# wenxichen/tensorflow_yolo2

Hardware: AMD Instinct MI355X
Metric: images/sec fwd+bwd Darknet-19 416x416 (higher is better)
Workload: dtype f16; 1 GPU; YOLO detector train step: darknet19_core + darknet19_detection(30) + get_loss + backward + Adam; image_size=416, batch_per_gpu=64, global_batch=64, S=13, B=2, parallelism=dp1, grad_allreduce=none

## Files before the change

include/yolo2_hip.h:

```cpp
#ifndef YOLO2_HIP_H
#define YOLO2_HIP_H
#include <stddef.h>
#include <stdint.h>

#ifdef __cplusplus
extern "C" {
#endif
#pragma GCC visibility push(default)

typedef struct y2_ctx y2_ctx;

#define Y2_F32 0
#define Y2_F16 1
#define Y2_BF16 2
#define Y2_F16X2 3
#define Y2_F16X2F 4
#define Y2_FP8 5

#define Y2_TAIL_NONE 0
#define Y2_TAIL_AVGPOOL 1

#define Y2_OK 0
#define Y2_ERR_ARG -1
#define Y2_ERR_HIP -2
// ... 177 lines not shown
int y2_momentum_step_packed(y2_ctx* ctx, float* accum, void* ctrl, float lr, float momentum, float grad_mult,
                            void* stream);

#define Y2_POLICY_CONSTANT 0
#define Y2_POLICY_STEPS 1
#define Y2_POLICY_POLY 2
#define Y2_SOLVER_MAX_STEPS 8
typedef struct y2_sgd_solver {
    float learning_rate, momentum, decay;
    int policy, burn_in, power, max_batches, nsteps;
    int steps[Y2_SOLVER_MAX_STEPS];
    float scales[Y2_SOLVER_MAX_STEPS];
} y2_sgd_solver;
int y2_solver_rate(const y2_sgd_solver* solver, int t, float* rate);
int y2_sgd_step(y2_ctx* ctx, float* accum, void* ctrl, int step, const y2_sgd_solver* solver, float grad_mult,
                void* stream);
int y2_sgd_step_packed(y2_ctx* ctx, float* accum, void* ctrl, int step, const y2_sgd_solver* solver, float grad_mult,
                       void* stream);

int y2_backward_adam(y2_ctx* ctx, const float* dout, float* m, float* v, void* ctrl, int step, float lr, float beta1,
                     float beta2, float eps, float grad_mult, void* stream);
int y2_backward_momentum(y2_ctx* ctx, const float* dout, float* accum, void* ctrl, float lr, float momentum,
                         float grad_mult, void* stream);

size_t y2_conv2d_workspace_bytes(int N, int H, int W, int Cin, int Cout, int k, int dtype);
int y2_conv2d(const float* x, const float* w, const float* bias, float* y, int N, int H, int W, int Cin,
              int Cout, int k, int dtype, void* workspace, void* stream);
int y2_conv2d_backward(const float* x, const float* w, const float* dy, float* dx, float* dw, int N, int H,
                       int W, int Cin, int Cout, int k, int dtype, void* workspace, void* stream);

#define Y2_LAUNCH_LOG_INTS 7
int y2_launch_log_enable(int enable);
int y2_launch_log_read(int* out, int max_records);

int y2_mx_quantize(const float* x, size_t rows, int C, uint8_t* q, uint8_t* scales, void* stream);

#define Y2_RESIZE_MAX_OUT_W 1024
int y2_resize_bilinear_u8_batch(const uint8_t* pool, const int64_t* table, const int32_t* index, int n, int out_h,
                                int out_w, uint8_t* out, void* stream);
int y2_letterbox_geometry(int im_h, int im_w, int size, int* geometry);
int y2_letterbox_u8_batch(const uint8_t* pool, const int64_t* table, const int32_t* index, int n, int size, int fill,
                          uint8_t* out, void* stream);
int y2_encode_labels(const double* boxes, const int32_t* counts, const int64_t* table, const int32_t* index, int n,
                     int max_obj, int image_size, int S, int num_class, float* labels, void* stream);

int y2_augment_u8_batch(const uint8_t* pool, const int64_t* table, const int32_t* index, const double* params, int n,
// ... 71 lines not shown
```

tensorflow_yolo2_amd/_lib.py:

```python
import ctypes as C
import os

_HERE = os.path.dirname(os.path.abspath(__file__))
LIB_PATH = os.path.join(_HERE, "libyolo2_hip.so")
if os.environ.get("Y2_DEV_LIB") == "1":
    LIB_PATH = os.path.join(_HERE, "libyolo2_hip_dev.so")
if os.environ.get("Y2_LIB_PATH"):
    LIB_PATH = os.environ["Y2_LIB_PATH"]

Y2_F32, Y2_F16, Y2_BF16, Y2_F16X2, Y2_F16X2F, Y2_FP8 = 0, 1, 2, 3, 4, 5
LOSS_SCALED = (Y2_F16, Y2_F16X2, Y2_F16X2F)
Y2_TAIL_NONE, Y2_TAIL_AVGPOOL = 0, 1
LAUNCH_LOG_INTS = 7
DTYPES = {"f32": Y2_F32, "fp32": Y2_F32, "float32": Y2_F32,
          "f16": Y2_F16, "fp16": Y2_F16, "float16": Y2_F16,
          "bf16": Y2_BF16, "bfloat16": Y2_BF16,
          "f16x2": Y2_F16X2,
          "f16x2f": Y2_F16X2F,
          "fp8": Y2_FP8, "mxfp8": Y2_FP8}

_vp, _i, _f, _sz, _u64 = C.c_void_p, C.c_int, C.c_float, C.c_size_t, C.c_uint64
_pi = C.POINTER(C.c_int)
_psz = C.POINTER(C.c_size_t)

# ... 91 lines not shown
    "y2_fully_connected_backward": (_i, [_vp, _vp, _vp, _vp, _vp, _i, _i, _i, _i, _vp]),
    "y2_conv7x7s2": (_i, [_vp, _vp, _vp, _i, _i, _i, _i, _vp]),
    "y2_conv7x7s2_t": (_i, [_vp, _vp, _vp, _i, _i, _i, _i, _i, _vp]),
    "y2_conv7x7s2_backward_filter": (_i, [_vp, _vp, _vp, _i, _i, _i, _i, _vp]),
    "y2_conv7x7s2_backward_filter_t": (_i, [_vp, _vp, _vp, _i, _i, _i, _i, _i, _vp]),
    "y2_bias_relu": (_i, [_vp, _vp, _sz, _i, _i, _vp]),
    "y2_bias_relu_backward": (_i, [_vp, _vp, _vp, _vp, _sz, _i, _i, _vp]),
    "y2_dropout": (_i, [_vp, _vp, _sz, _f, _u64, _vp]),
    "y2_dropout_dev": (_i, [_vp, _vp, _sz, _f, _vp, _vp]),
    "y2_adam_step": (_i, [_vp, _vp, _vp, _vp, _sz, _i, _f, _f, _f, _f, _f, _vp]),
    "y2_momentum_step": (_i, [_vp, _vp, _vp, _sz, _f, _f, _f, _vp]),
    "y2_grad_check": (_i, [_vp, _vp, _vp]),
    "y2_grad_check_more": (_i, [_vp, _vp, _vp]),
    "y2_grad_check_full": (_i, [_vp, _sz, _vp, _vp]),
    "y2_adam_step_guarded": (_i, [_vp, _vp, _vp, _vp, _sz, _vp, _f, _f, _f, _f, _f, _vp]),
    "y2_momentum_step_guarded": (_i, [_vp, _vp, _vp, _sz, _vp, _f, _f, _f, _vp]),
    "y2_adam_step_packed": (_i, [_vp, _vp, _vp, _vp, _i, _f, _f, _f, _f, _f, _vp]),
    "y2_momentum_step_packed": (_i, [_vp, _vp, _vp, _f, _f, _f, _vp]),
    "y2_solver_rate": (_i, [_vp, _i, C.POINTER(C.c_float)]),
    "y2_sgd_step": (_i, [_vp, _vp, _vp, _i, _vp, _f, _vp]),
    "y2_sgd_step_packed": (_i, [_vp, _vp, _vp, _i, _vp, _f, _vp]),
    "y2_backward_adam": (_i, [_vp, _vp, _vp, _vp, _vp, _i, _f, _f, _f, _f, _f, _vp]),
    "y2_backward_momentum": (_i, [_vp, _vp, _vp, _vp, _f, _f, _f, _vp]),
    "y2_conv2d_workspace_bytes": (_sz, [_i, _i, _i, _i, _i, _i, _i]),
    "y2_conv2d": (_i, [_vp, _vp, _vp, _vp, _i, _i, _i, _i, _i, _i, _i, _vp, _vp]),
    "y2_conv2d_backward": (_i, [_vp, _vp, _vp, _vp, _vp, _i, _i, _i, _i, _i, _i, _i, _vp, _vp]),
    "y2_launch_log_enable": (_i, [_i]),
    "y2_launch_log_read": (_i, [_pi, _i]),
    "y2_mx_quantize": (_i, [_vp, _sz, _i, _vp, _vp, _vp]),
    "y2_resize_bilinear_u8_batch": (_i, [_vp, _vp, _vp, _i, _i, _i, _vp, _vp]),
    "y2_letterbox_geometry": (_i, [_i, _i, _i, _pi]),
    "y2_letterbox_u8_batch": (_i, [_vp, _vp, _vp, _i, _i, _i, _vp, _vp]),
    "y2_encode_labels": (_i, [_vp, _vp, _vp, _vp, _i, _i, _i, _i, _i, _vp, _vp]),
    "y2_augment_u8_batch": (_i, [_vp, _vp, _vp, _vp, _i, _i, _i, _i, _vp, _vp]),
    "y2_encode_labels_window": (_i, [_vp, _vp, _vp, _vp, _vp, _i, _i, _i, _i, _i, _vp, _vp]),
    "y2_encode_box_list": (_i, [_vp, _vp, _vp, _vp, _vp, _i, _i, _i, _i, _vp, _vp, _vp]),
    "y2_encode_box_list_draw": (_i, [_vp, _vp, _vp, _vp, _vp, _vp, _i, _i, _i, _i, _vp, _vp, _vp]),
    "y2_warp_u8_batch": (_i, [_vp, _vp, _vp, _vp, _vp, _i, _i, _i, _i, _vp, _vp, _vp]),
    "y2_detect_grid_batch": (_i, [_vp, _vp, _vp, _i, _i, _i, _i, _f, _f, _i, _vp, _vp, _vp, _vp]),
    "y2_detect_anchor_batch": (_i, [_vp, _vp, _vp, _vp, _i, _i, _i, _i, _f, _f, _i, _vp, _vp, _vp, _vp]),
    "y2_detect_anchor_batch_lb": (_i, [_vp, _vp, _vp, _vp, _i, _i, _i, _i, _f, _f, _i, _i, _vp, _vp, _vp, _vp]),
    "y2_detect_anchor_classes_batch": (_i, [_vp, _vp, _vp, _vp, _i, _i, _i, _i, _f, _f, _i, _vp, _vp, _vp, _vp]),
    "y2_detect_anchor_classes_batch_lb": (_i, [_vp, _vp, _vp, _vp, _i, _i, _i, _i, _f, _f, _i, _i, _vp, _vp, _vp, _vp]),
    "y2_voc_match_batch": (_i, [_vp, _vp, _vp, _vp, _vp, _vp, _vp, _i, _i, _i, _f, _vp, _vp]),
    "y2_letterbox_darknet_batch": (_i, [_vp, _vp, _vp, _i, _i, _vp, _vp]),
    "y2_detect_anchor_classes_batch_dk": (_i, [_vp, _vp, _vp, _vp, _i, _i, _i, _i, _f, _f, _i, _i, _vp, _vp, _vp, _vp]),
# ... 62 lines not shown
```

tensorflow_yolo2_amd/csrc/kernels.h:

```cpp
#pragma once
#include <hip/hip_runtime.h>
#include <stddef.h>
#include <stdint.h>
#include <atomic>
#include "../../include/yolo2_hip.h"

namespace y2 {

inline size_t dtype_size(int dtype) { return (dtype == 0 || dtype >= 3) ? 4 : 2; }
inline int dtype_kbytes(int dtype) { return dtype == 0 ? 4 : 2; }
inline bool dtype_split(int dtype) { return dtype >= 3; }
inline int dtype_plain(int dtype) { return dtype >= 3 ? 0 : dtype; }

struct ConvArgs {
    const void* x;
    const void* w;
    void* y;
    const float* bias;
    float* part_cnt;
    float* part_mean;
    float* part_m2;
    int N, H, W, C;
    int M;
    int Cout;
// ... 357 lines not shown
hipError_t launch_pack_input_u8(int dtype, const uint8_t* img, void* x4, int N, int H, int W, hipStream_t s);
hipError_t launch_pack_weights(int dtype, const float* W, void* wf, void* wd, int taps, int Cin, int Cout,
                               int Cout_pad, int Kc, int Cin_pad, int Cdy, int frag, hipStream_t s);
hipError_t launch_pack_conv1_weights(int dtype, const float* W, void* wp, hipStream_t s);
struct PackLayer {
    const float* W;
    size_t w_off;
    void* wf;
    void* wd;
    int taps, Cin, Cout, Cout_pad, Kc, Cin_pad, Cdy;
    int wf_bx, wf_by, wf_blocks, wd_blocks, first_block;
    int opt_first;
    int wf_frag, wd_frag;
};
void pack_layer_plan(PackLayer& L, int first_block, int elem_size);
hipError_t launch_pack_all(int dtype, const PackLayer* tab_dev, int nlayers, int total_blocks, hipStream_t s);
struct OptPackArgs {
    float* p; float* slot0; float* slot1; const float* g;
    const void* ctrl;
    float lr_t, b1, b2, eps, gmult;
    int kind;
    const PackLayer* tab; int nlayers; int tile_blocks;
    const unsigned* small; int nsmall;
};
hipError_t launch_opt_pack(int dtype, const OptPackArgs& a, hipStream_t s);
hipError_t launch_convert_grad(int dtype, const float* src, void* dst, int M, int C, int ldd, float scale,
                               hipStream_t s);
hipError_t launch_unpack_act(int dtype, const void* xp, float* out, int N, int H, int W, int C, int Cs,
                             hipStream_t s);
hipError_t launch_pack_act_region(int dtype, const float* in, void* region, size_t region_bytes, size_t front_px, int N,
                                  int H, int W, int C, int Cs, hipStream_t s);
hipError_t launch_pack_act(int dtype, const float* in, void* xp, int N, int H, int W, int C, int Cs,
                           hipStream_t s);
hipError_t launch_cast_to_f32(int dtype, const void* src, float* dst, size_t rows, int C, int lds, hipStream_t s,
                              float scale = 1.0f);

struct BnFinalizeArgs {
    const float* part_cnt;
    const float* part_mean;
    const float* part_m2;
    int P, C, ldp;
    const float* gamma;
    const float* beta;
    float* moving_mean;
    float* moving_var;
    float* scale;
// ... 78 lines not shown
    float lambda_coord, lambda_noobj;
};
int loss_blocks(int N, int S);
hipError_t launch_yolo_loss(const LossArgs& a, hipStream_t s);
hipError_t launch_get_iou(const float* b1, const float* b2, float* out, int n, hipStream_t s);
hipError_t launch_decode(const float* pred, int S, int B, int C, int im_w, int im_h, float thresh, int* out,
                         float* out_conf, hipStream_t s);
hipError_t launch_avgpool_fwd(const float* h, float* out, int N, int H, int W, int C, int k, hipStream_t s);
hipError_t launch_avgpool_bwd(const float* dout, float* dh, int N, int H, int W, int C, int k, hipStream_t s);
hipError_t launch_softmax_ce(const float* logits, const int* labels, float* loss, float* dlogits, int N, int C,
                             hipStream_t s);

hipError_t launch_accuracy(const float* logits, const int* labels, float* acc, int N, int C, hipStream_t s);

hipError_t launch_adam(float* p, float* m, float* v, const float* g, size_t n, float lr_t, float b1, float b2,
                       float eps, float gscale, hipStream_t s);
hipError_t launch_momentum(float* p, float* acc, const float* g, size_t n, float lr, float mom, float gscale,
                           hipStream_t s);
hipError_t launch_grad_check(const float* g, size_t n, void* ctrl, hipStream_t s);
hipError_t launch_grad_check_ranges(const float* g, const void* ranges_dev, int nranges, void* ctrl, hipStream_t s,
                                    unsigned* flag = nullptr, bool keep = false);
hipError_t launch_range_check(const float* x, size_t n, float limit, void* ctrl, hipStream_t s);
hipError_t launch_opt_ctrl_advance(void* ctrl, float lr, float b1, float b2, hipStream_t s);
hipError_t launch_adam_guarded(float* p, float* m, float* v, const float* g, size_t n, const void* ctrl, float b1,
                               float b2, float eps, float gscale, hipStream_t s);
hipError_t launch_momentum_guarded(float* p, float* acc, const float* g, size_t n, const void* ctrl, float lr, float mom,
                                   float gscale, hipStream_t s);
struct SgdSeg { unsigned off, cnt, first_block, decayed; };
int sgd_seg_blocks(size_t off, size_t cnt);
hipError_t launch_sgd(float* p, float* acc, const float* g, const SgdSeg* segs_dev, int nsegs, int blocks,
                      const void* ctrl, float lr_t, float mom, float decay, float gscale, hipStream_t s);
hipError_t launch_sgd_ctrl_advance(void* ctrl, const y2_sgd_solver& sv, hipStream_t s);
hipError_t launch_init_trunc_normal(float* p, size_t n, float stddev, uint64_t seed, uint64_t stream_id,
                                    hipStream_t s);
hipError_t launch_fill(float* p, size_t n, float v, hipStream_t s);

constexpr int kDetectMaxCand = Y2_DETECT_MAX_CANDIDATES;
constexpr int kDetectAnchorMaxCand = Y2_DETECT_ANCHOR_MAX_CANDIDATES;
constexpr int kMatchMaxObj = Y2_MATCH_MAX_OBJECTS;

void* op_scratch(hipStream_t s, size_t bytes);
int op_scratch_error();

}
```

tensorflow_yolo2_amd/csrc/net.hip:

```cpp
#include <math.h>
#include <stdarg.h>
#include <stdio.h>
#include <string.h>

#include <algorithm>
#include <string>
#include <vector>

#include "../../include/yolo2_hip.h"
#include "common.h"
#include "kernels.h"
#include "optim_math.h"

using namespace y2;

static thread_local std::string g_err;
namespace y2 {
int set_error(int code, const char* msg) {
    g_err = msg;
    return code;
}
}
static int fail(int code, const char* fmt, ...) {
    char buf[512];
// ... 129 lines not shown
    size_t o_ks = 0, ks_floats = 0;
    size_t o_gram = 0;
    size_t slab_floats = 0;
    int n_chkranges = 0, n_smallranges = 0, opt_tile_blocks = 0;
    int n_chk_upper = 0, n_small_upper = 0;
    int n_sgdsegs = 0, sgd_blocks = 0;
    struct FusedOpt {
        bool on = false;
        int kind = 0;
        float* slot0 = nullptr; float* slot1 = nullptr;
        void* ctrl = nullptr;
        float lr = 0.f, b1 = 0.f, b2 = 0.f, eps = 0.f, gmult = 1.f;
        int step = 0;
    } fopt;
    std::vector<PackLayer> packtab;
    std::vector<BnInferLayer> infertab;
    std::vector<SgdSeg> sgdsegs;
    int pack_blocks = 0;
    int prof = 0;
    struct ProfRec { int cat, layer; hipEvent_t a, b; };
    int prof_layer = -1;
    hipStream_t side = nullptr;
    hipEvent_t ev_fork = nullptr, ev_join = nullptr;
    std::vector<hipEvent_t> mark_main, mark_side;
    int n_marks = 0;
    const int* cur_marks = nullptr;
    float* dinput = nullptr;
    void* ext_xin = nullptr;
    void* ext_out = nullptr;
    const void* ext_join = nullptr;
    int ext_join_self = 0;
    const void* ext_dout = nullptr;
    void* ext_dx = nullptr;
    std::vector<ProfRec> prof_recs;
    size_t prof_used = 0;
    size_t sz() const { return dtype_size(dtype); }
    PadGeom in_geom(int l) const { return PadGeom{N, L[l].H, L[l].W, L[l].cin_s}; }
    PadGeom dy_geom(int l) const { return PadGeom{N, L[l].H, L[l].W, L[l].ldy}; }
    Conv1Plan conv1_plan(bool trains, bool training) const {
        const Layer& y = L[0];
        return plan_conv1(dtype, bwd_dtype, N, y.H, y.W, y.pool, y.cout, y.ldy, trains, L.size() > 1, training);
    }
};

enum { CAT_CONV_FWD = 0, CAT_CONV1_FWD, CAT_DGRAD, CAT_WGRAD, CAT_CONV1_WGRAD, CAT_BN_FWD, CAT_BN_BWD, CAT_MISC,
       CAT_COUNT };
// ... 381 lines not shown
        if (tail_k <= 0 || last.Ho < tail_k || last.Wo < tail_k) {
            delete c;
            return fail(Y2_ERR_ARG, "avgpool window %d does not fit %dx%d", tail_k, last.Ho, last.Wo);
        }
        c->outN = batch; c->outH = last.Ho / tail_k; c->outW = last.Wo / tail_k; c->outC = last.cout;
    } else {
        c->outN = batch; c->outH = last.Ho; c->outW = last.Wo; c->outC = last.cout;
    }
    if (last.pool) {
        delete c;
        return fail(Y2_ERR_ARG, "the last layer must not pool");
    }
    plan(c);
    *out = c;
    return Y2_OK;
}

void y2_ctx_destroy(y2_ctx* ctx) {
    if (!ctx) return;
    for (auto& r : ctx->prof_recs) { (void)hipEventDestroy(r.a); (void)hipEventDestroy(r.b); }
    if (ctx->side) (void)hipStreamDestroy(ctx->side);
    if (ctx->ev_fork) (void)hipEventDestroy(ctx->ev_fork);
    if (ctx->ev_join) (void)hipEventDestroy(ctx->ev_join);
    for (auto e : ctx->mark_main) (void)hipEventDestroy(e);
    for (auto e : ctx->mark_side) (void)hipEventDestroy(e);
    delete ctx;
}

int y2_profile_enable(y2_ctx* c, int on) {
    if (on == 1 || on == 2) c->prof_used = 0;
    c->prof = on == 3 ? 2 : on;
    return Y2_OK;
}
int y2_profile_collect(y2_ctx* c, double* ms, int* count, int ncat) {
    if (ncat < CAT_COUNT) return fail(Y2_ERR_ARG, "need room for %d categories", (int)CAT_COUNT);
    for (int i = 0; i < ncat; ++i) { ms[i] = 0.0; count[i] = 0; }
    for (size_t i = 0; i < c->prof_used; ++i) {
        auto& r = c->prof_recs[i];
        HIPCHK(hipEventSynchronize(r.b));
        float t = 0.f;
        HIPCHK(hipEventElapsedTime(&t, r.a, r.b));
        ms[r.cat] += t;
        count[r.cat] += 1;
    }
    c->prof_used = 0;
    return Y2_OK;
// ... 76 lines not shown
    c->packtab.clear();
    int nb = 0, ntile = 0;
    for (size_t l = 0; l < c->L.size(); ++l) {
        Layer& y = c->L[l];
        if (y.first3) continue;
        PackLayer p{};
        p.W = params + y.pW;
        p.w_off = y.pW;
        p.wf = c->ws + y.wf;
        p.wd = training ? (void*)(c->ws + y.wd) : nullptr;
        p.taps = y.k * y.k; p.Cin = y.cin; p.Cout = y.cout; p.Cout_pad = y.cout_pad; p.Kc = y.cin_s;
        p.Cin_pad = y.cin_pad; p.Cdy = y.ldy;
        const int split = dtype_split(c->dtype) ? 1 : 0;
        p.wf_frag = y.wf_frag = plan_conv(c->dtype, fwd_args(c, (int)l, false, FOLD_NONE)).filter_layout;
        p.wd_frag = y.wd_frag = plan_conv(dgrad_dtype(c, (int)l), dgrad_args(c, (int)l, false, false)).filter_layout;
        pack_layer_plan(p, nb, split ? 2 : (int)c->sz());
        nb += p.wf_blocks + p.wd_blocks;
        p.opt_first = ntile;
        ntile += p.wf_blocks;
        c->packtab.push_back(p);
    }
    c->pack_blocks = nb;
    c->opt_tile_blocks = ntile;
    {
        std::vector<unsigned> rg;
        for (size_t l = 1; l <= c->L.size(); ++l) {
            const Layer& y = c->L[l % c->L.size()];
            rg.push_back((unsigned)y.pb);
            rg.push_back((unsigned)(3 * y.cout));
            rg.push_back(0u);
        }
        c->n_small_upper = (int)c->L.size() - 1;
        if (c->L[0].first3) {
            rg.push_back((unsigned)c->L[0].pW);
            rg.push_back((unsigned)(27 * c->L[0].cout));
            rg.push_back(1u);
        }
        c->n_smallranges = (int)(rg.size() / 3);
        HIPCHK(hipMemcpyAsync(c->ws + c->o_smallranges, rg.data(), rg.size() * sizeof(unsigned), hipMemcpyHostToDevice,
                              (hipStream_t)stream));
    }
    {
        std::vector<SgdSeg>& sg = c->sgdsegs;
        sg.clear();
        unsigned nblk = 0;
        for (const Layer& y : c->L) {
// ... 302 lines not shown
        HIPCHK(launch_avgpool_fwd((const float*)(c->ws + c->o_h32), out, c->N, y.Ho, y.Wo, y.cout, c->tail_k, s));
    }
    c->fwd_saved = true;
    c->moving_pending = !update_moving;
    return Y2_OK;
}

int y2_update_moving_stats(y2_ctx* c, void* stream) {
    if (!c->ws) return fail(Y2_ERR_STATE, "bind buffers first");
    if (!c->fwd_saved) return fail(Y2_ERR_STATE, "run y2_forward first");
    if (!c->moving_pending) return Y2_OK;
    hipStream_t s = (hipStream_t)stream;
    for (size_t l = 0; l < c->L.size(); ++l) {
        if (!c->fwd.L[l].training) continue;
        const Layer& y = c->L[l];
        const float* stat = (const float*)(c->ws + y.stat);
        HIPCHK(launch_bn_update_moving(stat + 2 * y.ldy, stat + 6 * y.ldy, c->state + y.smm, c->state + y.smv, y.cout,
                                       c->bn_momentum, s));
    }
    c->moving_pending = false;
    return Y2_OK;
}

static int fused_opt_part(y2_ctx* c, int part, hipStream_t s);

int y2_backward(y2_ctx* c, const float* dout, int layer_lo, int layer_hi, void* stream) {
    if (c->fp8) return fail(Y2_ERR_STATE, "Y2_FP8 contexts are inference only: no backward pass (create the context with another dtype to train)");
    if (!c->ws || !c->bound_training) return fail(Y2_ERR_STATE, "bind with training=1 first");
    if (!c->fwd_saved) return fail(Y2_ERR_STATE, "run y2_forward before y2_backward");
    const int nl = (int)c->L.size();
    if (layer_lo < 0 || layer_hi > nl || layer_lo >= layer_hi) return fail(Y2_ERR_ARG, "bad layer range");
    hipStream_t s = (hipStream_t)stream;
    const size_t sz = c->sz();
    const float inv_gs = 1.0f / c->grad_scale;
    char* dA[2] = {c->ws + c->o_dA0, c->ws + c->o_dA1};
    const bool ext_top = layer_hi == nl && c->ext_dout != nullptr;
    if (layer_hi == nl) c->dA_half = 0;
    if (ext_top) {
        c->dA_cur = 0;
        if (layer_lo > 0 && c->grads) HIPCHK(hipMemsetAsync(c->grads, 0, c->L[layer_lo].pW * sizeof(float), s));
    } else if (layer_hi == nl) {
        if (!dout) return fail(Y2_ERR_ARG, "null output gradient");
        const Layer& y = c->L.back();
        const float* src = dout;
        if (c->tail == Y2_TAIL_AVGPOOL) {
            float* dh = (float*)(c->ws + c->o_dh32);
            HIPCHK(launch_avgpool_bwd(dout, dh, c->N, y.Ho, y.Wo, y.cout, c->tail_k, s));
            src = dh;
        }
        c->dA_cur = 0;
        PROF(CAT_MISC);
        HIPCHK(launch_convert_grad(c->dtype, src, dA[0], y.M, y.cout, y.ldy, c->grad_scale, s));
        if (layer_lo > 0 && c->grads) HIPCHK(hipMemsetAsync(c->grads, 0, c->L[layer_lo].pW * sizeof(float), s));
    }
    float* psum = (float*)(c->ws + c->o_psum);
    bool forked = false;
    bool opt_early = false;
    const NetPlan n = plan_net(c, c->fwd.train_core, c->fwd.train_head, layer_lo, layer_hi);
    const Conv1Plan& p1 = n.c1;
    if (!c->side && std::any_of(n.L.begin(), n.L.end(), [](const LayerPlan& p) { return p.wgrad_side; })) {
        HIPCHK(hipStreamCreateWithFlags(&c->side, hipStreamNonBlocking));
        HIPCHK(hipEventCreateWithFlags(&c->ev_fork, hipEventDisableTiming));
        HIPCHK(hipEventCreateWithFlags(&c->ev_join, hipEventDisableTiming));
    }
    for (int l = layer_hi - 1; l >= layer_lo; --l) {
        c->prof_layer = l;
        const Layer& y = c->L[l];
        const LayerPlan& p = n.L[l];
        float* stat = (float*)(c->ws + y.stat);
        char* dyp = c->ws + y.dyp + c->dy_geom(l).base_off(sz);
        BnBwdArgs b{};
        b.dA = (ext_top && l == nl - 1) ? c->ext_dout : (const void*)dA[c->dA_cur]; b.y = c->ws + y.y;
        b.scale = stat; b.shift = stat + y.ldy; b.mean = stat + 2 * y.ldy; b.invstd = stat + 3 * y.ldy;
        b.coef = stat + 4 * y.ldy;
        b.psum = psum;
        b.dgamma = c->grads + y.pg; b.dbeta = c->grads + y.pbeta; b.dbias = c->grads + y.pb;
        b.dyp = dyp;
        b.N = c->N; b.H = y.H; b.W = y.W; b.C = y.cout; b.ldy = y.ldy;
        b.ldd = y.ldy;
        b.pool = y.pool; b.training = p.training; b.inv_grad_scale = inv_gs;
        b.P = p.bP;
        b.slope = y.slope;
        b.hi_only = (c->bwd_dtype == 4 && !y.first3) ? 1 : 0;
        b.dA_half = c->dA_half;
        if (c->zero_bias_grad) b.dbias = nullptr;
        const int bn_dtype = y.first3 ? dtype_plain(c->dtype) : c->dtype;
        if (p.bred == BR_CONV1_LIN && c->fopt.on && forked && l == 0) {
            HIPCHK(hipEventRecord(c->ev_fork, s));
            HIPCHK(hipStreamWaitEvent(c->side, c->ev_fork, 0));
            const int rc = fused_opt_part(c, 1, c->side);
            if (rc != Y2_OK) return rc;
            opt_early = true;
        }
        {
            PROF(CAT_BN_BWD);
            if (p.bred == BR_CONV1_LIN) {
                Conv1WgradLinArgs g{};
                g.x4 = c->ws + y.xin + c->in_geom(l).base_off(sz); g.dA = b.dA;
                if (p1.keep == C1K_IDX3) {
                    g.idx3 = (const unsigned*)(c->ws + y.idx0); g.Wf = c->params + y.pW; g.bias = c->params + y.pb;
                } else {
                    g.ysel = c->ws + y.ysel;
                    g.idx = (const unsigned short*)(c->ws + y.idx0);
                }
                g.scale = b.scale; g.shift = b.shift; g.acc = (float*)(c->ws + c->o_lin); g.psum = psum;
                g.N = c->N; g.H = y.H; g.W = y.W;
                HIPCHK(launch_conv1_wgrad_lin(p1, g, s));
            } else if (p.bred == BR_CONV1_RECOMPUTE) {
                Conv1BnBwdArgs q{};
                q.x4 = c->ws + y.xin + c->in_geom(l).base_off(sz); q.w = c->ws + y.wf; q.bias = c->params + y.pb;
                q.scale = b.scale; q.shift = b.shift; q.dA = b.dA; q.psum = psum;
                q.N = c->N; q.H = y.H; q.W = y.W;
                HIPCHK(launch_conv1_bnbwd_reduce(p1, q, s));
            } else if (p.bred == BR_KERNEL) {
// ... 22 lines not shown
            g.N = c->N; g.H = y.H; g.W = y.W; g.inv_grad_scale = inv_gs;
            HIPCHK(hipMemsetAsync(g.dW, 0, (size_t)27 * y.cout * sizeof(float), s));
            { PROF(CAT_CONV1_WGRAD); HIPCHK(launch_conv1_wgrad_fused(p1, g, s)); }
        } else if (p.wgrad == WG_CONV1) {
            Conv1WgradArgs g{};
            g.x4 = xin; g.dy = dyp; g.dW = c->grads + y.pW;
            g.N = c->N; g.H = y.H; g.W = y.W; g.M = y.M; g.scale = inv_gs;
            HIPCHK(hipMemsetAsync(g.dW, 0, (size_t)27 * y.cout * sizeof(float), s));
            { PROF(CAT_CONV1_WGRAD); HIPCHK(launch_conv1_wgrad(p1, g, s)); }
        } else {
            WgradArgs g{};
            g.x = xin; g.dy = dyp; g.dW = c->grads + y.pW;
            g.N = c->N; g.H = y.H; g.W = y.W; g.M = y.M;
            g.Cin = y.cin_s; g.Cdy = y.ldy; g.Cout = y.cout; g.taps = y.k * y.k; g.splitk = 0; g.scale = inv_gs;
            g.slab = (float*)(c->ws + c->o_slab); g.slab_floats = c->slab_floats;
            hipStream_t ws_ = s;
            if (p.wgrad_side) {
                HIPCHK(hipEventRecord(c->ev_fork, s));
                HIPCHK(hipStreamWaitEvent(c->side, c->ev_fork, 0));
                ws_ = c->side;
                forked = true;
            }
            { ProfScope _p(c, ws_, CAT_WGRAD); HIPCHK(launch_wgrad_auto(c->bwd_dtype, g, ws_)); }
            if (p.dgrad) {
                ConvArgs a = dgrad_args(c, l, p.dgrad_fuse, p.dgrad_guard);
                a.y = (l == 0 && c->ext_dx) ? (char*)c->ext_dx : dA[c->dA_cur ^ 1];
                { PROF(CAT_DGRAD); HIPCHK(launch_conv(p.dgrad_dtype, a, s, y.wd_frag)); }
                c->dA_cur ^= 1;
                c->dA_half = p.dgrad_dtype == 5 ? 1 : 0;
                if (l == 0 && c->dinput)
                    HIPCHK(launch_cast_to_f32(c->dtype, c->ext_dx ? (const void*)c->ext_dx : (const void*)dA[c->dA_cur], c->dinput,
                                              (size_t)y.M, y.cin, y.cin, s, inv_gs));
            }
        }
        for (int k = 0; k < c->n_marks; ++k)
            if (c->cur_marks[k] == l) {
                HIPCHK(hipEventRecord(c->mark_main[k], s));
                HIPCHK(hipEventRecord(c->mark_side[k], forked ? c->side : s));
            }
    }
    if (forked) {
        HIPCHK(hipEventRecord(c->ev_join, c->side));
        HIPCHK(hipStreamWaitEvent(s, c->ev_join, 0));
    }
    if (c->fopt.on) return fused_opt_part(c, opt_early ? 2 : 0, s);
    return Y2_OK;
}

int y2_backward_marks(y2_ctx* c, const float* dout, int n_marks, const int* mark_layers, void* stream) {
    if (n_marks < 0 || (n_marks > 0 && !mark_layers)) return fail(Y2_ERR_ARG, "bad marks");
    for (int k = 0; k < n_marks; ++k)
        if (mark_layers[k] < 0 || mark_layers[k] >= (int)c->L.size())
            return fail(Y2_ERR_ARG, "mark %d: layer %d out of range", k, mark_layers[k]);
    while ((int)c->mark_main.size() < n_marks) {
        hipEvent_t a = nullptr, b = nullptr;
        HIPCHK(hipEventCreateWithFlags(&a, hipEventDisableTiming));
        HIPCHK(hipEventCreateWithFlags(&b, hipEventDisableTiming));
        c->mark_main.push_back(a);
        c->mark_side.push_back(b);
    }
    c->n_marks = n_marks;
    c->cur_marks = mark_layers;
    const int rc = y2_backward(c, dout, 0, (int)c->L.size(), stream);
    c->n_marks = 0;
    c->cur_marks = nullptr;
    return rc;
}
int y2_backward_input(y2_ctx* c, const float* dout, float* dinput, void* stream) {
// ... 152 lines not shown
    HIPCHK(launch_grad_check(grads, n, ctrl, (hipStream_t)stream));
    return Y2_OK;
}
int y2_range_check(const float* x, size_t n, float limit, void* ctrl, void* stream) {
    if (!x || !ctrl || !(limit > 0.f)) return fail(Y2_ERR_ARG, "bad arguments");
    if (n) HIPCHK(launch_range_check(x, n, limit, ctrl, (hipStream_t)stream));
    return Y2_OK;
}
int y2_adam_step_guarded(float* params, float* m, float* v, const float* grads, size_t n, void* ctrl, float lr,
                         float beta1, float beta2, float eps, float grad_mult, void* stream) {
    if (!params || !m || !v || !grads || !ctrl) return fail(Y2_ERR_ARG, "bad arguments");
    HIPCHK(launch_opt_ctrl_advance(ctrl, lr, beta1, beta2, (hipStream_t)stream));
    HIPCHK(launch_adam_guarded(params, m, v, grads, n, ctrl, beta1, beta2, eps, grad_mult, (hipStream_t)stream));
    return Y2_OK;
}
int y2_momentum_step_guarded(float* params, float* accum, const float* grads, size_t n, void* ctrl, float lr,
                             float momentum, float grad_mult, void* stream) {
    if (!params || !accum || !grads || !ctrl) return fail(Y2_ERR_ARG, "bad arguments");
    HIPCHK(launch_opt_ctrl_advance(ctrl, lr, 0.9f, 0.999f, (hipStream_t)stream));
    HIPCHK(launch_momentum_guarded(params, accum, grads, n, ctrl, lr, momentum, grad_mult, (hipStream_t)stream));
    return Y2_OK;
}
static int opt_step_packed(y2_ctx* c, int kind, float* slot0, float* slot1, void* ctrl, float lr_t_or_lr, float b1,
                           float b2, float eps, float grad_mult, hipStream_t s, int part = 0) {
    if (!c->ws || !c->grads || !c->bound_training) return fail(Y2_ERR_STATE, "bind with training=1 first");
    OptPackArgs a{};
    a.p = c->params; a.slot0 = slot0; a.slot1 = slot1; a.g = c->grads; a.ctrl = ctrl;
    a.lr_t = lr_t_or_lr; a.b1 = b1; a.b2 = b2; a.eps = eps; a.gmult = grad_mult; a.kind = kind;
    a.tab = (const PackLayer*)(c->ws + c->o_packtab); a.nlayers = (int)c->packtab.size();
    a.tile_blocks = part == 2 ? 0 : c->opt_tile_blocks;
    const unsigned* small = (const unsigned*)(c->ws + c->o_smallranges);
    a.small = part == 2 ? small + 3 * c->n_small_upper : small;
    a.nsmall = part == 0 ? c->n_smallranges : (part == 1 ? c->n_small_upper : c->n_smallranges - c->n_small_upper);
    HIPCHK(launch_opt_pack(c->dtype, a, s));
    if (part != 1 && !c->L.empty() && c->L[0].first3)
        HIPCHK(launch_pack_conv1_weights(c->dtype, c->params + c->L[0].pW, c->ws + c->L[0].wf, s));
    if (part != 1) c->weights_dirty = false;
    return Y2_OK;
}
static int fused_opt_part(y2_ctx* c, int part, hipStream_t s) {
    const y2_ctx::FusedOpt& f = c->fopt;
    double lr_t = f.lr;
    if (f.ctrl) {
        if (part != 2) {
            const bool upper = part == 1;
            HIPCHK(launch_grad_check_ranges(c->grads, c->ws + c->o_chkranges, upper ? c->n_chk_upper : c->n_chkranges,
                                            f.ctrl, s, upper ? (unsigned*)(c->ws + c->o_nfflag) : nullptr));
            HIPCHK(launch_opt_ctrl_advance(f.ctrl, f.lr, f.kind == 0 ? f.b1 : 0.9f, f.kind == 0 ? f.b2 : 0.999f, s));
        }
    } else if (f.kind == 0) {
        lr_t = (double)f.lr * sqrt(1.0 - pow((double)f.b2, f.step)) / (1.0 - pow((double)f.b1, f.step));
    }
    return opt_step_packed(c, f.kind, f.slot0, f.slot1, f.ctrl, (float)lr_t, f.b1, f.b2, f.eps, f.gmult, s, part);
}
int y2_backward_adam(y2_ctx* c, const float* dout, float* m, float* v, void* ctrl, int step, float lr, float beta1,
                     float beta2, float eps, float grad_mult, void* stream) {
    if (c->fp8) return fail(Y2_ERR_STATE, "Y2_FP8 contexts are inference only: no backward pass (create the context with another dtype to train)");
    if (!m || !v || (!ctrl && step < 1)) return fail(Y2_ERR_ARG, "bad arguments");
    if (!c->grads) return fail(Y2_ERR_STATE, "bind with a gradient buffer first");
    c->fopt = y2_ctx::FusedOpt{true, 0, m, v, ctrl, lr, beta1, beta2, eps, grad_mult, step};
    const int rc = y2_backward(c, dout, 0, (int)c->L.size(), stream);
    c->fopt.on = false;
    return rc;
}
int y2_backward_momentum(y2_ctx* c, const float* dout, float* accum, void* ctrl, float lr, float momentum,
                         float grad_mult, void* stream) {
    if (c->fp8) return fail(Y2_ERR_STATE, "Y2_FP8 contexts are inference only: no backward pass (create the context with another dtype to train)");
    if (!accum) return fail(Y2_ERR_ARG, "bad arguments");
    if (!c->grads) return fail(Y2_ERR_STATE, "bind with a gradient buffer first");
    c->fopt = y2_ctx::FusedOpt{true, 1, accum, nullptr, ctrl, lr, momentum, 0.f, 0.f, grad_mult, 0};
    const int rc = y2_backward(c, dout, 0, (int)c->L.size(), stream);
    c->fopt.on = false;
    return rc;
}
int y2_adam_step_packed(y2_ctx* c, float* m, float* v, void* ctrl, int step, float lr, float beta1, float beta2,
                        float eps, float grad_mult, void* stream) {
    if (!m || !v || (!ctrl && step < 1)) return fail(Y2_ERR_ARG, "bad arguments");
    double lr_t = lr;
    if (ctrl && step >= 0) HIPCHK(launch_opt_ctrl_advance(ctrl, lr, beta1, beta2, (hipStream_t)stream));
    else if (!ctrl) lr_t = (double)lr * sqrt(1.0 - pow((double)beta2, step)) / (1.0 - pow((double)beta1, step));
    return opt_step_packed(c, 0, m, v, ctrl, (float)lr_t, beta1, beta2, eps, grad_mult, (hipStream_t)stream);
}
int y2_momentum_step_packed(y2_ctx* c, float* accum, void* ctrl, float lr, float momentum, float grad_mult,
                            void* stream) {
    if (!accum) return fail(Y2_ERR_ARG, "bad arguments");
    if (ctrl) HIPCHK(launch_opt_ctrl_advance(ctrl, lr, 0.9f, 0.999f, (hipStream_t)stream));
    return opt_step_packed(c, 1, accum, nullptr, ctrl, lr, momentum, 0.f, 0.f, grad_mult, (hipStream_t)stream);
// ... 223 lines not shown
```

tensorflow_yolo2_amd/csrc/optim.hip:

```cpp
#include "common.h"
#include "kernels.h"
#include "optim_math.h"

namespace y2 {

__global__ void adam_kernel(float4* p, float4* m, float4* v, const float4* g, size_t n4, float lr_t, float b1,
                            float b2, float eps, float gscale, float* pt, float* mt, float* vt, const float* gt,
                            size_t tail0, size_t n) {
    for (size_t i = (size_t)blockIdx.x * blockDim.x + threadIdx.x; i < n4; i += (size_t)gridDim.x * blockDim.x) {
        float4 pp = p[i], mm = m[i], vv = v[i], gg = g[i];
        float* P = &pp.x; float* M = &mm.x; float* V = &vv.x; const float* G = &gg.x;
#pragma unroll
        for (int k = 0; k < 4; ++k) adam_update(P[k], M[k], V[k], G[k] * gscale, lr_t, b1, b2, eps);
        p[i] = pp; m[i] = mm; v[i] = vv;
    }
    if (blockIdx.x == 0) {
        for (size_t i = tail0 + threadIdx.x; i < n; i += blockDim.x) {
            float pk = pt[i], mk = mt[i], vk = vt[i];
            adam_update(pk, mk, vk, gt[i] * gscale, lr_t, b1, b2, eps);
            mt[i] = mk; vt[i] = vk; pt[i] = pk;
        }
    }
}
hipError_t launch_adam(float* p, float* m, float* v, const float* g, size_t n, float lr_t, float b1, float b2,
// ... 84 lines not shown
hipError_t launch_grad_check_ranges(const float* g, const void* ranges_dev, int nranges, void* ctrl, hipStream_t s,
                                    unsigned* flag, bool keep) {
    if (!keep) {
        hipError_t e = hipMemsetAsync(ctrl, 0, sizeof(int), s);
        if (e != hipSuccess) return e;
    }
    const int nb = nranges < 1 ? 1 : (nranges < 64 ? nranges : 64);
    hipLaunchKernelGGL(grad_check_ranges_kernel, dim3(nb), dim3(256), 0, s, g, (const unsigned*)ranges_dev, nranges,
                       (OptCtrl*)ctrl, flag);
    return hipGetLastError();
}

__global__ void opt_ctrl_advance_kernel(OptCtrl* ctrl, float lr, float b1, float b2) {
    if (ctrl->found_inf) {
        ctrl->skipped += 1;
    } else {
        const int t = ctrl->step + 1;
        ctrl->step = t;
        ctrl->lr_t = (float)((double)lr * sqrt(1.0 - pow((double)b2, (double)t)) / (1.0 - pow((double)b1, (double)t)));
    }
}
hipError_t launch_opt_ctrl_advance(void* ctrl, float lr, float b1, float b2, hipStream_t s) {
    hipLaunchKernelGGL(opt_ctrl_advance_kernel, dim3(1), dim3(1), 0, s, (OptCtrl*)ctrl, lr, b1, b2);
    return hipGetLastError();
}

__global__ void adam_guarded_kernel(float4* p, float4* m, float4* v, const float4* g, size_t n4, const OptCtrl* ctrl,
                                    float b1, float b2, float eps, float gscale, float* pt, float* mt, float* vt,
                                    const float* gt, size_t tail0, size_t n) {
    if (ctrl->found_inf) return;
    const float lr_t = ctrl->lr_t;
    for (size_t i = (size_t)blockIdx.x * blockDim.x + threadIdx.x; i < n4; i += (size_t)gridDim.x * blockDim.x) {
        float4 pp = p[i], mm = m[i], vv = v[i], gg = g[i];
        float* P = &pp.x; float* M = &mm.x; float* V = &vv.x; const float* G = &gg.x;
#pragma unroll
        for (int k = 0; k < 4; ++k) adam_update(P[k], M[k], V[k], G[k] * gscale, lr_t, b1, b2, eps);
        p[i] = pp; m[i] = mm; v[i] = vv;
    }
    if (blockIdx.x == 0) {
        for (size_t i = tail0 + threadIdx.x; i < n; i += blockDim.x) {
            float pk = pt[i], mk = mt[i], vk = vt[i];
            adam_update(pk, mk, vk, gt[i] * gscale, lr_t, b1, b2, eps);
            mt[i] = mk; vt[i] = vk; pt[i] = pk;
        }
    }
}
// ... 136 lines not shown
```

tensorflow_yolo2_amd/csrc/pack.hip:

```cpp
#include "common.h"
#include "kernels.h"
#include "optim_math.h"

namespace y2 {

template <typename T>
__global__ void pack_input_kernel(const float* __restrict__ img, T* __restrict__ x4, int N, int H, int W) {
    const size_t total = (size_t)N * H * W;
    for (size_t p = (size_t)blockIdx.x * blockDim.x + threadIdx.x; p < total; p += (size_t)gridDim.x * blockDim.x) {
        const int w = (int)(p % W);
        const int h = (int)((p / W) % H);
        const int n = (int)(p / ((size_t)W * H));
        const float* s = img + p * 3;
        T* d = x4 + bpix(n, h, w, H, W) * 4;
        d[0] = Elem<T>::from_f32(s[0]);
        d[1] = Elem<T>::from_f32(s[1]);
        d[2] = Elem<T>::from_f32(s[2]);
        d[3] = Elem<T>::from_f32(1.f);
    }
}
template <typename T>
static hipError_t pack_input_T(const float* img, void* x4, int N, int H, int W, hipStream_t s) {
    size_t total = (size_t)N * H * W;
    size_t nb = (total + 255) / 256;
// ... 530 lines not shown

struct OptCtrlView { int found_inf, step, skipped, reserved; float lr_t; };

template <int KIND>
Y2_DEV void opt_update(float& p, float& s0, float& s1, float g, float lr_t, float b1, float b2, float eps,
                       bool decayed = true) {
    if (KIND == 0) adam_update(p, s0, s1, g, lr_t, b1, b2, eps);
    else if (KIND == 1) momentum_update(p, s0, g, lr_t, b1);
    else sgd_update(p, s0, g, lr_t, b1, b2, decayed);
}

template <typename T, int KIND, bool SPLIT = false>
__global__ __launch_bounds__(256) void opt_pack_kernel(OptPackArgs a) {
    constexpr int EPC = 16 / sizeof(T);
    constexpr int CPR = 64 / EPC;
    constexpr int RPP = 256 / CPR;
    float lr_t = a.lr_t;
    if (a.ctrl) {
        const OptCtrlView* c = (const OptCtrlView*)a.ctrl;
        if (c->found_inf) return;
        if (KIND != 1) lr_t = c->lr_t;
    }
    const int tid = threadIdx.x;
    const int b = blockIdx.x;
    if (b >= a.tile_blocks) {
        const int nb = gridDim.x - a.tile_blocks, bi = b - a.tile_blocks;
        for (int r = 0; r < a.nsmall; ++r) {
            const unsigned off = a.small[3 * r], cnt = a.small[3 * r + 1];
            const bool decayed = KIND == 2 && a.small[3 * r + 2] != 0;
            for (unsigned i = bi * 256 + tid; i < cnt; i += nb * 256) {
                float p = a.p[off + i], s0 = a.slot0[off + i], s1 = KIND == 0 ? a.slot1[off + i] : 0.f;
                opt_update<KIND>(p, s0, s1, a.g[off + i] * a.gmult, lr_t, a.b1, a.b2, a.eps, decayed);
                a.p[off + i] = p; a.slot0[off + i] = s0;
                if (KIND == 0) a.slot1[off + i] = s1;
            }
        }
        return;
    }
    __shared__ float tile[64][65];
    int l = 0;
    while (l + 1 < a.nlayers && b >= a.tab[l + 1].opt_first) ++l;
    const PackLayer L = a.tab[l];
    const int local = b - L.opt_first;
    const int bx = local % L.wf_bx, by = (local / L.wf_bx) % L.wf_by, t = local / (L.wf_bx * L.wf_by);
    const int ci0 = by * 64, co0 = bx * 64;
    const int c4 = (tid & 15) * 4, r0 = tid >> 4;
    const bool vec = (L.Cout & 3) == 0;
#pragma unroll
    for (int pass = 0; pass < 4; ++pass) {
        const int r = pass * 16 + r0;
        const int ci = ci0 + r, co = co0 + c4;
        float pv[4] = {0.f, 0.f, 0.f, 0.f};
        if (ci < L.Cin && co < L.Cout) {
            const size_t o = L.w_off + ((size_t)t * L.Cin + ci) * L.Cout + co;
            if (vec) {
                f32x4 p = *(const f32x4*)(a.p + o), s0 = *(const f32x4*)(a.slot0 + o), g = *(const f32x4*)(a.g + o);
                f32x4 s1 = KIND == 0 ? *(const f32x4*)(a.slot1 + o) : f32x4{0.f, 0.f, 0.f, 0.f};
#pragma unroll
                for (int k = 0; k < 4; ++k) {
                    float pk = p[k], ak = s0[k], bk = s1[k];
                    opt_update<KIND>(pk, ak, bk, g[k] * a.gmult, lr_t, a.b1, a.b2, a.eps);
                    p[k] = pk; s0[k] = ak; s1[k] = bk; pv[k] = pk;
// ... 122 lines not shown
```

Measured before the change: 7338 images/s.

## Run upper-layer optimizer tiles early on a low-priority stream during backward

Adds a dedicated low-priority optimizer stream. Once the upper layers' weight gradients are ready (after layer 2 wgrad), the packed optimizer update for all tiles except layer 1's runs on that stream, overlapping the remaining backward work. Only layer 1's tiles and the small ranges are left for the final launch, which first waits on the optimizer stream's event. It also fuses the grad-finite check and the ctrl step-advance into one single-block guard kernel, removing a launch. The cost is extra streams and events plus more complex cross-stream ordering of parameter updates.

```diff
diff --git a/include/yolo2_hip.h b/include/yolo2_hip.h
--- a/include/yolo2_hip.h
+++ b/include/yolo2_hip.h
@@ -223,6 +223,7 @@
                      float beta2, float eps, float grad_mult, void* stream);
 int y2_backward_momentum(y2_ctx* ctx, const float* dout, float* accum, void* ctrl, float lr, float momentum,
                          float grad_mult, void* stream);
+int y2_opt_schedule(const y2_ctx* ctx);
 
 size_t y2_conv2d_workspace_bytes(int N, int H, int W, int Cin, int Cout, int k, int dtype);
 int y2_conv2d(const float* x, const float* w, const float* bias, float* y, int N, int H, int W, int Cin,
diff --git a/tensorflow_yolo2_amd/_lib.py b/tensorflow_yolo2_amd/_lib.py
--- a/tensorflow_yolo2_amd/_lib.py
+++ b/tensorflow_yolo2_amd/_lib.py
@@ -137,6 +137,7 @@
     "y2_sgd_step_packed": (_i, [_vp, _vp, _vp, _i, _vp, _f, _vp]),
     "y2_backward_adam": (_i, [_vp, _vp, _vp, _vp, _vp, _i, _f, _f, _f, _f, _f, _vp]),
     "y2_backward_momentum": (_i, [_vp, _vp, _vp, _vp, _f, _f, _f, _vp]),
+    "y2_opt_schedule": (_i, [_vp]),
     "y2_conv2d_workspace_bytes": (_sz, [_i, _i, _i, _i, _i, _i, _i]),
     "y2_conv2d": (_i, [_vp, _vp, _vp, _vp, _i, _i, _i, _i, _i, _i, _i, _vp, _vp]),
     "y2_conv2d_backward": (_i, [_vp, _vp, _vp, _vp, _vp, _i, _i, _i, _i, _i, _i, _i, _vp, _vp]),
diff --git a/tensorflow_yolo2_amd/csrc/kernels.h b/tensorflow_yolo2_amd/csrc/kernels.h
--- a/tensorflow_yolo2_amd/csrc/kernels.h
+++ b/tensorflow_yolo2_amd/csrc/kernels.h
@@ -403,6 +403,7 @@
     int kind;
     const PackLayer* tab; int nlayers; int tile_blocks;
     const unsigned* small; int nsmall;
+    int tile_first;
 };
 hipError_t launch_opt_pack(int dtype, const OptPackArgs& a, hipStream_t s);
 hipError_t launch_convert_grad(int dtype, const float* src, void* dst, int M, int C, int ldd, float scale,
@@ -527,6 +528,8 @@
                                     unsigned* flag = nullptr, bool keep = false);
 hipError_t launch_range_check(const float* x, size_t n, float limit, void* ctrl, hipStream_t s);
 hipError_t launch_opt_ctrl_advance(void* ctrl, float lr, float b1, float b2, hipStream_t s);
+hipError_t launch_opt_guard(const float* g, const void* ranges_dev, int nranges, void* ctrl, unsigned* flag, float lr,
+                            float b1, float b2, hipStream_t s);
 hipError_t launch_adam_guarded(float* p, float* m, float* v, const float* g, size_t n, const void* ctrl, float b1,
                                float b2, float eps, float gscale, hipStream_t s);
 hipError_t launch_momentum_guarded(float* p, float* acc, const float* g, size_t n, const void* ctrl, float lr, float mom,
diff --git a/tensorflow_yolo2_amd/csrc/net.hip b/tensorflow_yolo2_amd/csrc/net.hip
--- a/tensorflow_yolo2_amd/csrc/net.hip
+++ b/tensorflow_yolo2_amd/csrc/net.hip
@@ -175,6 +175,10 @@
     int prof_layer = -1;
     hipStream_t side = nullptr;
     hipEvent_t ev_fork = nullptr, ev_join = nullptr;
+    hipStream_t opt = nullptr;
+    hipEvent_t ev_upper = nullptr, ev_opt = nullptr;
+    int opt_tiles_l1 = 0;
+    int opt_schedule = 0;
     std::vector<hipEvent_t> mark_main, mark_side;
     int n_marks = 0;
     const int* cur_marks = nullptr;
@@ -602,6 +606,9 @@
     if (ctx->side) (void)hipStreamDestroy(ctx->side);
     if (ctx->ev_fork) (void)hipEventDestroy(ctx->ev_fork);
     if (ctx->ev_join) (void)hipEventDestroy(ctx->ev_join);
+    if (ctx->opt) (void)hipStreamDestroy(ctx->opt);
+    if (ctx->ev_upper) (void)hipEventDestroy(ctx->ev_upper);
+    if (ctx->ev_opt) (void)hipEventDestroy(ctx->ev_opt);
     for (auto e : ctx->mark_main) (void)hipEventDestroy(e);
     for (auto e : ctx->mark_side) (void)hipEventDestroy(e);
     delete ctx;
@@ -724,6 +731,7 @@
     }
     c->pack_blocks = nb;
     c->opt_tile_blocks = ntile;
+    c->opt_tiles_l1 = c->L[0].first3 && !c->packtab.empty() ? c->packtab[0].wf_blocks : 0;
     {
         std::vector<unsigned> rg;
         for (size_t l = 1; l <= c->L.size(); ++l) {
@@ -1072,7 +1080,7 @@
     return Y2_OK;
 }
 
-static int fused_opt_part(y2_ctx* c, int part, hipStream_t s);
+static int fused_opt_part(y2_ctx* c, int part, hipStream_t s, int late_tiles);
 
 int y2_backward(y2_ctx* c, const float* dout, int layer_lo, int layer_hi, void* stream) {
     if (c->fp8) return fail(Y2_ERR_STATE, "Y2_FP8 contexts are inference only: no backward pass (create the context with another dtype to train)");
@@ -1113,6 +1121,17 @@
         HIPCHK(hipEventCreateWithFlags(&c->ev_fork, hipEventDisableTiming));
         HIPCHK(hipEventCreateWithFlags(&c->ev_join, hipEventDisableTiming));
     }
+    static const bool no_opt_early = getenv("Y2_NO_OPT_EARLY") != nullptr;
+    const bool opt3 = c->fopt.on && !no_opt_early && layer_lo == 0 && c->opt_tiles_l1 > 0 && p1.bwd == C1B_LINEAR && c->side;
+    if (opt3 && !c->opt) {
+        int least = 0, greatest = 0;
+        HIPCHK(hipDeviceGetStreamPriorityRange(&least, &greatest));
+        HIPCHK(hipStreamCreateWithPriority(&c->opt, hipStreamNonBlocking, least));
+        HIPCHK(hipEventCreateWithFlags(&c->ev_upper, hipEventDisableTiming));
+        HIPCHK(hipEventCreateWithFlags(&c->ev_opt, hipEventDisableTiming));
+    }
+    bool upper_recorded = false;
+    int late_tiles = 0;
     for (int l = layer_hi - 1; l >= layer_lo; --l) {
         c->prof_layer = l;
         const Layer& y = c->L[l];
@@ -1137,9 +1156,19 @@
         const int bn_dtype = y.first3 ? dtype_plain(c->dtype) : c->dtype;
         if (p.bred == BR_CONV1_LIN && c->fopt.on && forked && l == 0) {
             HIPCHK(hipEventRecord(c->ev_fork, s));
-            HIPCHK(hipStreamWaitEvent(c->side, c->ev_fork, 0));
-            const int rc = fused_opt_part(c, 1, c->side);
-            if (rc != Y2_OK) return rc;
+            if (opt3) {
+                if (!upper_recorded) HIPCHK(hipEventRecord(c->ev_upper, c->side));
+                HIPCHK(hipStreamWaitEvent(c->opt, c->ev_fork, 0));
+                HIPCHK(hipStreamWaitEvent(c->opt, c->ev_upper, 0));
+                const int rc = fused_opt_part(c, 1, c->opt, c->opt_tiles_l1);
+                if (rc != Y2_OK) return rc;
+                HIPCHK(hipEventRecord(c->ev_opt, c->opt));
+                late_tiles = c->opt_tiles_l1;
+            } else {
+                HIPCHK(hipStreamWaitEvent(c->side, c->ev_fork, 0));
+                const int rc = fused_opt_part(c, 1, c->side, 0);
+                if (rc != Y2_OK) return rc;
+            }
             opt_early = true;
         }
         {
@@ -1208,6 +1237,10 @@
                 forked = true;
             }
             { ProfScope _p(c, ws_, CAT_WGRAD); HIPCHK(launch_wgrad_auto(c->bwd_dtype, g, ws_)); }
+            if (opt3 && l == 2 && forked) {
+                HIPCHK(hipEventRecord(c->ev_upper, c->side));
+                upper_recorded = true;
+            }
             if (p.dgrad) {
                 ConvArgs a = dgrad_args(c, l, p.dgrad_fuse, p.dgrad_guard);
                 a.y = (l == 0 && c->ext_dx) ? (char*)c->ext_dx : dA[c->dA_cur ^ 1];
@@ -1229,7 +1262,9 @@
         HIPCHK(hipEventRecord(c->ev_join, c->side));
         HIPCHK(hipStreamWaitEvent(s, c->ev_join, 0));
     }
-    if (c->fopt.on) return fused_opt_part(c, opt_early ? 2 : 0, s);
+    if (late_tiles) HIPCHK(hipStreamWaitEvent(s, c->ev_opt, 0));
+    if (c->fopt.on) c->opt_schedule = late_tiles ? 2 : opt_early ? 1 : 0;
+    if (c->fopt.on) return fused_opt_part(c, opt_early ? 2 : 0, s, late_tiles);
     return Y2_OK;
 }
 
@@ -1428,13 +1463,15 @@
     return Y2_OK;
 }
 static int opt_step_packed(y2_ctx* c, int kind, float* slot0, float* slot1, void* ctrl, float lr_t_or_lr, float b1,
-                           float b2, float eps, float grad_mult, hipStream_t s, int part = 0) {
+                           float b2, float eps, float grad_mult, hipStream_t s, int part = 0, int late_tiles = 0) {
     if (!c->ws || !c->grads || !c->bound_training) return fail(Y2_ERR_STATE, "bind with training=1 first");
     OptPackArgs a{};
     a.p = c->params; a.slot0 = slot0; a.slot1 = slot1; a.g = c->grads; a.ctrl = ctrl;
     a.lr_t = lr_t_or_lr; a.b1 = b1; a.b2 = b2; a.eps = eps; a.gmult = grad_mult; a.kind = kind;
     a.tab = (const PackLayer*)(c->ws + c->o_packtab); a.nlayers = (int)c->packtab.size();
-    a.tile_blocks = part == 2 ? 0 : c->opt_tile_blocks;
+    if (late_tiles < 0 || late_tiles > c->opt_tile_blocks) return fail(Y2_ERR_STATE, "optimizer tile split out of range");
+    a.tile_first = part == 1 ? late_tiles : 0;
+    a.tile_blocks = part == 2 ? late_tiles : c->opt_tile_blocks - a.tile_first;
     const unsigned* small = (const unsigned*)(c->ws + c->o_smallranges);
     a.small = part == 2 ? small + 3 * c->n_small_upper : small;
     a.nsmall = part == 0 ? c->n_smallranges : (part == 1 ? c->n_small_upper : c->n_smallranges - c->n_small_upper);
@@ -1444,20 +1481,27 @@
     if (part != 1) c->weights_dirty = false;
     return Y2_OK;
 }
-static int fused_opt_part(y2_ctx* c, int part, hipStream_t s) {
+static int fused_opt_part(y2_ctx* c, int part, hipStream_t s, int late_tiles) {
+    static const bool no_guard_fuse = getenv("Y2_NO_GUARD_FUSE") != nullptr;
     const y2_ctx::FusedOpt& f = c->fopt;
     double lr_t = f.lr;
     if (f.ctrl) {
         if (part != 2) {
             const bool upper = part == 1;
-            HIPCHK(launch_grad_check_ranges(c->grads, c->ws + c->o_chkranges, upper ? c->n_chk_upper : c->n_chkranges,
-                                            f.ctrl, s, upper ? (unsigned*)(c->ws + c->o_nfflag) : nullptr));
-            HIPCHK(launch_opt_ctrl_advance(f.ctrl, f.lr, f.kind == 0 ? f.b1 : 0.9f, f.kind == 0 ? f.b2 : 0.999f, s));
+            const int nr = upper ? c->n_chk_upper : c->n_chkranges;
+            unsigned* flag = upper ? (unsigned*)(c->ws + c->o_nfflag) : nullptr;
+            const float b1 = f.kind == 0 ? f.b1 : 0.9f, b2 = f.kind == 0 ? f.b2 : 0.999f;
+            if (late_tiles && !no_guard_fuse) {
+                HIPCHK(launch_opt_guard(c->grads, c->ws + c->o_chkranges, nr, f.ctrl, flag, f.lr, b1, b2, s));
+            } else {
+                HIPCHK(launch_grad_check_ranges(c->grads, c->ws + c->o_chkranges, nr, f.ctrl, s, flag));
+                HIPCHK(launch_opt_ctrl_advance(f.ctrl, f.lr, b1, b2, s));
+            }
         }
     } else if (f.kind == 0) {
         lr_t = (double)f.lr * sqrt(1.0 - pow((double)f.b2, f.step)) / (1.0 - pow((double)f.b1, f.step));
     }
-    return opt_step_packed(c, f.kind, f.slot0, f.slot1, f.ctrl, (float)lr_t, f.b1, f.b2, f.eps, f.gmult, s, part);
+    return opt_step_packed(c, f.kind, f.slot0, f.slot1, f.ctrl, (float)lr_t, f.b1, f.b2, f.eps, f.gmult, s, part, late_tiles);
 }
 int y2_backward_adam(y2_ctx* c, const float* dout, float* m, float* v, void* ctrl, int step, float lr, float beta1,
                      float beta2, float eps, float grad_mult, void* stream) {
@@ -1469,6 +1513,7 @@
     c->fopt.on = false;
     return rc;
 }
+int y2_opt_schedule(const y2_ctx* c) { return c ? c->opt_schedule : 0; }
 int y2_backward_momentum(y2_ctx* c, const float* dout, float* accum, void* ctrl, float lr, float momentum,
                          float grad_mult, void* stream) {
     if (c->fp8) return fail(Y2_ERR_STATE, "Y2_FP8 contexts are inference only: no backward pass (create the context with another dtype to train)");
diff --git a/tensorflow_yolo2_amd/csrc/optim.hip b/tensorflow_yolo2_amd/csrc/optim.hip
--- a/tensorflow_yolo2_amd/csrc/optim.hip
+++ b/tensorflow_yolo2_amd/csrc/optim.hip
@@ -130,6 +130,37 @@
 }
 hipError_t launch_opt_ctrl_advance(void* ctrl, float lr, float b1, float b2, hipStream_t s) {
     hipLaunchKernelGGL(opt_ctrl_advance_kernel, dim3(1), dim3(1), 0, s, (OptCtrl*)ctrl, lr, b1, b2);
+    return hipGetLastError();
+}
+
+__global__ __launch_bounds__(1024) void opt_guard_kernel(const float* g, const unsigned* ranges, int nranges, OptCtrl* ctrl,
+                                                         unsigned* flag, float lr, float b1, float b2) {
+    unsigned bad = 0;
+    if (flag && threadIdx.x == 0) {
+        bad = *flag != 0;
+        *flag = 0;
+    }
+    for (int r = 0; r < nranges; ++r) {
+        const float* p = g + ranges[2 * r];
+        const unsigned cnt = ranges[2 * r + 1];
+        for (unsigned i = threadIdx.x; i < cnt; i += blockDim.x)
+            bad |= (__float_as_uint(p[i]) & 0x7F800000u) == 0x7F800000u;
+    }
+    const int any = __syncthreads_or(bad != 0);
+    if (threadIdx.x != 0) return;
+    ctrl->found_inf = any ? 1 : 0;
+    if (any) {
+        ctrl->skipped += 1;
+    } else {
+        const int t = ctrl->step + 1;
+        ctrl->step = t;
+        ctrl->lr_t = (float)((double)lr * sqrt(1.0 - pow((double)b2, (double)t)) / (1.0 - pow((double)b1, (double)t)));
+    }
+}
+hipError_t launch_opt_guard(const float* g, const void* ranges_dev, int nranges, void* ctrl, unsigned* flag, float lr,
+                            float b1, float b2, hipStream_t s) {
+    hipLaunchKernelGGL(opt_guard_kernel, dim3(1), dim3(1024), 0, s, g, (const unsigned*)ranges_dev, nranges,
+                       (OptCtrl*)ctrl, flag, lr, b1, b2);
     return hipGetLastError();
 }
 
diff --git a/tensorflow_yolo2_amd/csrc/pack.hip b/tensorflow_yolo2_amd/csrc/pack.hip
--- a/tensorflow_yolo2_amd/csrc/pack.hip
+++ b/tensorflow_yolo2_amd/csrc/pack.hip
@@ -576,9 +576,8 @@
         if (KIND != 1) lr_t = c->lr_t;
     }
     const int tid = threadIdx.x;
-    const int b = blockIdx.x;
-    if (b >= a.tile_blocks) {
-        const int nb = gridDim.x - a.tile_blocks, bi = b - a.tile_blocks;
+    if ((int)blockIdx.x >= a.tile_blocks) {
+        const int nb = gridDim.x - a.tile_blocks, bi = blockIdx.x - a.tile_blocks;
         for (int r = 0; r < a.nsmall; ++r) {
             const unsigned off = a.small[3 * r], cnt = a.small[3 * r + 1];
             const bool decayed = KIND == 2 && a.small[3 * r + 2] != 0;
@@ -592,6 +591,7 @@
         return;
     }
     __shared__ float tile[64][65];
+    const int b = blockIdx.x + a.tile_first;
     int l = 0;
     while (l + 1 < a.nlayers && b >= a.tab[l + 1].opt_first) ++l;
     const PackLayer L = a.tab[l];
```

Measured after the change: 7333 images/s. No clear change (-0.1%).
